# funcwj/setk

Measured on AMD Instinct MI355X. Metric: real-time-factor (audio-sec/wall-sec), 8-ch 16 kHz MVDR, higher is better.
Workload: dtype f32; 1 GPU; 8-ch 16 kHz oracle-mask MVDR, 30 s utterances, 125 per GPU (BASELINE configs[2] shard: 1000 at 8 GPUs), STFT 512/256/hann/center, inputs resident in HBM; utts_per_gpu=125, channels=8, frames=1876, beamformer=mvdr, parallelism=utterance-sharded x1

## Files before the change

setk_amd/csrc/fft512.h:

```cpp
#pragma once
#include <hip/hip_runtime.h>

namespace setk {

typedef float2 cf;

#define SETK_DEV __device__ __forceinline__

#define SETK_GLOBAL __attribute__((address_space(1)))
typedef const SETK_GLOBAL float* gcfloat_p;
typedef float v2f __attribute__((ext_vector_type(2)));
typedef const SETK_GLOBAL v2f* gcfloat2_p;
template <class T>
SETK_DEV const SETK_GLOBAL T* gptr(const T* p) {
    return (const SETK_GLOBAL T*)p;
}

SETK_DEV cf cadd(cf a, cf b) { return make_float2(a.x + b.x, a.y + b.y); }
SETK_DEV cf csub(cf a, cf b) { return make_float2(a.x - b.x, a.y - b.y); }
SETK_DEV cf cmul(cf a, cf b) {
    return make_float2(a.x * b.x - a.y * b.y, a.x * b.y + a.y * b.x);
}
SETK_DEV cf cmulc(cf a, cf b) {
    return make_float2(a.x * b.x + a.y * b.y, a.y * b.x - a.x * b.y);
}
SETK_DEV cf cconj(cf a) { return make_float2(a.x, -a.y); }
SETK_DEV cf cscale(cf a, float s) { return make_float2(a.x * s, a.y * s); }

__host__ __device__ constexpr int dft16_pos(int q) { return (q >> 2) + 4 * (q & 3); }

template <int DIR>
SETK_DEV void dft4(cf& a, cf& b, cf& c, cf& d) {
    cf s0 = cadd(a, c), s1 = csub(a, c), s2 = cadd(b, d), s3 = csub(b, d);
    cf r3 = DIR < 0 ? make_float2(s3.y, -s3.x) : make_float2(-s3.y, s3.x);
    a = cadd(s0, s2);
    c = csub(s0, s2);
    b = cadd(s1, r3);
    d = csub(s1, r3);
}

template <int DIR, int M>
SETK_DEV cf twid16(cf v) {
    constexpr float C1 = 0.92387953251128673848f;
    constexpr float S1 = 0.38268343236508978178f;
    constexpr float R2 = 0.70710678118654752440f;
    constexpr float D = (float)DIR;
    if constexpr (M == 1) return cmul(v, make_float2(C1, D * S1));
    if constexpr (M == 2) return make_float2(R2 * (v.x - D * v.y), R2 * (D * v.x + v.y));
    if constexpr (M == 3) return cmul(v, make_float2(S1, D * C1));
    if constexpr (M == 4) return make_float2(-D * v.y, D * v.x);
    if constexpr (M == 6) return make_float2(R2 * (-v.x - D * v.y), R2 * (D * v.x - v.y));
    if constexpr (M == 9) return cmul(v, make_float2(-C1, -D * S1));
    return v;
}

template <int DIR>
SETK_DEV void dft16(cf (&v)[16]) {
#pragma unroll
    for (int b = 0; b < 4; ++b) dft4<DIR>(v[b], v[4 + b], v[8 + b], v[12 + b]);
    v[4 * 1 + 1] = twid16<DIR, 1>(v[4 * 1 + 1]);
    v[4 * 2 + 1] = twid16<DIR, 2>(v[4 * 2 + 1]);
    v[4 * 3 + 1] = twid16<DIR, 3>(v[4 * 3 + 1]);
    v[4 * 1 + 2] = twid16<DIR, 2>(v[4 * 1 + 2]);
    v[4 * 2 + 2] = twid16<DIR, 4>(v[4 * 2 + 2]);
    v[4 * 3 + 2] = twid16<DIR, 6>(v[4 * 3 + 2]);
    v[4 * 1 + 3] = twid16<DIR, 3>(v[4 * 1 + 3]);
    v[4 * 2 + 3] = twid16<DIR, 6>(v[4 * 2 + 3]);
    v[4 * 3 + 3] = twid16<DIR, 9>(v[4 * 3 + 3]);
#pragma unroll
    for (int c = 0; c < 4; ++c)
        dft4<DIR>(v[4 * c], v[4 * c + 1], v[4 * c + 2], v[4 * c + 3]);
}

constexpr int kRow5 = 10;
__host__ __device__ constexpr int slot_entries(int row) { return 16 * row; }
__host__ __device__ constexpr int table_entries(int row) {
    return (row % 2 == 0) ? 2 * 16 * row + 16 * kRow5 : 640;
}
template <int ROW> struct LaneTab {
    static constexpr bool rows = (ROW % 2 == 0);
    static constexpr int estride = rows ? 1 : 16;
    static constexpr int lstride = rows ? ROW : 1;
    static constexpr int lstride5 = rows ? kRow5 : 1;
    static constexpr int size = rows ? 16 * ROW : 256;
};

template <int N, bool WIDE = true>
SETK_DEV void lds_row(const cf* row, cf (&out)[N]) {
    if (WIDE) {
        const float4* r4 = reinterpret_cast<const float4*>(__builtin_assume_aligned(row, 16));
#pragma unroll
        for (int n = 0; n < N / 2; ++n) {
            const float4 t = r4[n];
            out[2 * n] = make_float2(t.x, t.y);
            out[2 * n + 1] = make_float2(t.z, t.w);
        }
    } else {
#pragma unroll
        for (int n = 0; n < N; ++n) out[n] = row[n];
    }
}

template <int ROW>
SETK_DEV void fill_lane_tables(cf* win_l, cf* tw_l, cf* tw5_l, const float* window,
                               const float2* tw256, const float2* tw512, int tid, int nthreads) {
    for (int i = tid; i < 256; i += nthreads) {
        const int la = i & 15, j = i >> 4, n = la + 16 * j;
        typedef LaneTab<ROW> L;
        win_l[la * L::lstride + j * L::estride] = make_float2(window[2 * n], window[2 * n + 1]);
        tw_l[la * L::lstride + j * L::estride] = tw256[j * 16 + la];
    }
    for (int i = tid; i < 128; i += nthreads) {
        const int la = i & 15, m = i >> 4;
        tw5_l[la * LaneTab<ROW>::lstride5 + m * LaneTab<ROW>::estride] = tw512[la + 16 * m];
    }
}

template <int ROW>
SETK_DEV void apply_window(cf (&v)[16], const cf* win_row) {
    if (LaneTab<ROW>::rows) {
        const float4* w4 = reinterpret_cast<const float4*>(__builtin_assume_aligned(win_row, 16));
#pragma unroll
        for (int j = 0; j < 16; j += 2) {
            const float4 w = w4[j / 2];
            v[j] = make_float2(v[j].x * w.x, v[j].y * w.y);
            v[j + 1] = make_float2(v[j + 1].x * w.z, v[j + 1].y * w.w);
        }
    } else {
#pragma unroll
        for (int j = 0; j < 16; ++j) {
            const cf w = win_row[j * 16];
            v[j] = make_float2(v[j].x * w.x, v[j].y * w.y);
        }
    }
}

template <int DIR, int ROW, bool WIDE = (ROW % 2 == 0)>
SETK_DEV void fft256_stage_a_pad(cf (&v)[16], cf* slot, const cf* tw_row, int la) {
    dft16<DIR>(v);
    cf* dst = slot + la;
    if (WIDE) {
        const float4* w4 = reinterpret_cast<const float4*>(__builtin_assume_aligned(tw_row, 16));
#pragma unroll
        for (int q = 0; q < 16; q += 2) {
            const float4 w = w4[q / 2];
            cf t0 = v[dft16_pos(q)], t1 = v[dft16_pos(q + 1)];
            if (q) t0 = cmul(t0, make_float2(w.x, DIR > 0 ? -w.y : w.y));
            t1 = cmul(t1, make_float2(w.z, DIR > 0 ? -w.w : w.w));
            dst[q * ROW] = t0;
            dst[(q + 1) * ROW] = t1;
        }
    } else {
        cf wq[16];
        wq[1] = tw_row[16];
        wq[2] = tw_row[32];
#pragma unroll
        for (int q = 0; q < 16; ++q) {
            if (q + 3 < 16) wq[q + 3] = tw_row[(q + 3) * 16];
            cf t = v[dft16_pos(q)];
            if (q) {
                cf w = wq[q];
                if (DIR > 0) w.y = -w.y;
                t = cmul(t, w);
            }
            dst[q * ROW] = t;
        }
    }
}

template <int DIR, int ROW, bool WIDE = (ROW % 2 == 0)>
SETK_DEV void fft256_stage_b_pad(cf (&v)[16], const cf* slot, int la) {
    lds_row<16, WIDE>(slot + la * ROW, v);
    dft16<DIR>(v);
}

SETK_DEV void rfft_split(cf Zk, cf Zm, cf w, cf& Xk, cf& Xm) {
    cf A = make_float2(Zk.x + Zm.x, Zk.y - Zm.y);
    cf O = make_float2(Zk.y + Zm.y, Zm.x - Zk.x);
    cf B = cmul(w, O);
    Xk = cadd(A, B);
    Xm = make_float2(A.x - B.x, -(A.y - B.y));
}

SETK_DEV void irfft_merge(cf Yk, cf Ym, cf w, cf& Zk, cf& Zm) {
    cf E = make_float2(Yk.x + Ym.x, Yk.y - Ym.y);
    cf D = make_float2(Yk.x - Ym.x, Yk.y + Ym.y);
    cf O = cmulc(D, w);
    Zk = make_float2(E.x - O.y, E.y + O.x);
    Zm = make_float2(E.x + O.y, -E.y + O.x);
}

constexpr int kFrame = 512;

SETK_DEV int reflect_index(int i, int n) {
    if (i < 0) i = -i;
    if (i >= n) i = 2 * (n - 1) - i;
    return i;
}

template <class FloatPtr> struct RawPair;
template <> struct RawPair<gcfloat_p> {
    typedef gcfloat2_p ptr;
    static SETK_DEV cf get(ptr p, int i) {
        const v2f d = p[i];
        return make_float2(d.x, d.y);
    }
};
template <> struct RawPair<const float*> {
    typedef const float2* ptr;
    static SETK_DEV cf get(ptr p, int i) { return p[i]; }
};

template <class FloatPtr>
SETK_DEV void load_raw(cf (&v)[16], FloatPtr x, int n_samp, int s, int la, bool valid) {
    if (!valid) {
#pragma unroll
        for (int j = 0; j < 16; ++j) v[j] = make_float2(0.f, 0.f);
        return;
    }
    const bool interior = (s >= 0) && (s + kFrame <= n_samp) && ((((uintptr_t)(x + s)) & 7) == 0);
    if (interior) {
        typename RawPair<FloatPtr>::ptr p = (typename RawPair<FloatPtr>::ptr)(x + s);
#pragma unroll
        for (int j = 0; j < 16; ++j) v[j] = RawPair<FloatPtr>::get(p, la + 16 * j);
    } else {
#pragma unroll
        for (int j = 0; j < 16; ++j) {
            const int n = la + 16 * j;
            v[j] = make_float2(x[reflect_index(s + 2 * n, n_samp)],
                               x[reflect_index(s + 2 * n + 1, n_samp)]);
        }
    }
}

typedef const SETK_GLOBAL short* gcshort_p;
typedef const SETK_GLOBAL int* gcint_p;
SETK_DEV void load_raw_pcm(int (&v)[16], gcshort_p x, int n_samp, int s, int la, bool valid) {
    if (!valid) {
#pragma unroll
        for (int j = 0; j < 16; ++j) v[j] = 0;
        return;
    }
    const bool interior = (s >= 0) && (s + kFrame <= n_samp) && ((((uintptr_t)(x + s)) & 3) == 0);
    if (interior) {
        gcint_p p = (gcint_p)(x + s);
#pragma unroll
        for (int j = 0; j < 16; ++j) v[j] = p[la + 16 * j];
    } else {
#pragma unroll
        for (int j = 0; j < 16; ++j) {
            const int n = la + 16 * j;
            const int lo = x[reflect_index(s + 2 * n, n_samp)];
            const int hi = x[reflect_index(s + 2 * n + 1, n_samp)];
            v[j] = (lo & 0xffff) | (hi << 16);
        }
    }
}
SETK_DEV cf unpack_pcm(int v) { return make_float2((float)(short)(v & 0xffff), (float)(v >> 16)); }

SETK_DEV float qr_partner(float x) {
    int v = __builtin_bit_cast(int, x);
    v = __builtin_amdgcn_update_dpp(0, v, 0x140, 0xf, 0xf, true);
    v = __builtin_amdgcn_update_dpp(0, v, 0x121, 0xf, 0xf, true);
    return __builtin_bit_cast(float, v);
}

template <int ROW, bool WIDE = (ROW % 2 == 0)>
SETK_DEV void qr_stage23(cf* slot, float* nyq, const cf* tw5_row, int la) {
    cf v[16];
    fft256_stage_b_pad<-1, ROW, WIDE>(v, slot, la);
    const bool lane0 = (la == 0);
    cf* lo = slot + la;
    cf* mir = slot + (256 - 16 * 7) - la;
    cf t5[8];
    if (WIDE) {
        lds_row<8, true>(tw5_row, t5);
    } else {
        t5[0] = tw5_row[0];
        t5[1] = tw5_row[16];
    }
#pragma unroll
    for (int m = 0; m < 8; ++m) {
        if (!WIDE && m + 2 < 8) t5[m + 2] = tw5_row[16 * (m + 2)];
        const cf Zk = v[dft16_pos(m)];
        const cf src = v[dft16_pos(15 - m)];
        cf Zm = make_float2(qr_partner(src.x), qr_partner(src.y));
        const cf own = v[dft16_pos((16 - m) & 15)];
        Zm.x = lane0 ? own.x : Zm.x;
        Zm.y = lane0 ? own.y : Zm.y;
        cf Xk, Xm;
        rfft_split(Zk, Zm, t5[m], Xk, Xm);
        if (m == 0) {
            const cf Z128 = v[dft16_pos(8)];
            if (lane0) {
                slot[0] = make_float2(Xk.x, 0.f);
                *nyq = Xm.x;
                slot[128] = make_float2(2.f * Z128.x, -2.f * Z128.y);
            } else {
                lo[16 * m] = Xk;
                mir[16 * (7 - m)] = Xm;
            }
        } else {
            lo[16 * m] = Xk;
            mir[16 * (7 - m)] = Xm;
        }
    }
}

}
```

setk_amd/csrc/pass1.hip:

```cpp
#include "common.h"
#include "fft512.h"
#include "covar_fold.h"
#include <cstdio>
#include <type_traits>
#include <cstdlib>

namespace setk {

template <int C, bool DUMP, bool PCM = false>
__global__ __launch_bounds__(1024, 4) void stft_covar_kernel(Pass1Args a) {
    constexpr int NT = 1024;
    constexpr int TB = pass1_tile_frames(C);
    constexpr int NF = TB * C;
    constexpr int NP = npairs(C);
    constexpr int ND = PairSplit<C>::ND, NO = PairSplit<C>::NO;
    constexpr int NS = 32 / NF;
    constexpr int F = kBins, FP = kBinsPad;
    constexpr int ROW = 17;
    constexpr int SL = slot_entries(ROW);

    extern __shared__ __attribute__((aligned(16))) char smem[];
    cf* xt0 = reinterpret_cast<cf*>(smem);
    cf* win_l = xt0 + 2 * NF * SL;
    cf* tw_l = win_l + LaneTab<ROW>::size;
    cf* tw5_l = tw_l + LaneTab<ROW>::size;
    float* xn0 = reinterpret_cast<float*>(win_l + table_entries(ROW));
    float* nym = xn0 + 64;
    float* red = nym + 32;

    const int tid = threadIdx.x;
    const int wave = __builtin_amdgcn_readfirstlane(tid >> 6);
    const WorkItem wi = a.items[blockIdx.x];
    const UttDesc ud = a.utts[wi.utt];
    const int n_samp = ud.num_samples;
    const int T = ud.num_frames;
    const bool clamp = (a.flags & 0x2) != 0;
    const bool has_mn = ud.mask_n != nullptr;

    fill_lane_tables<ROW>(win_l, tw_l, tw5_l, a.window, a.tw256, a.tw512, tid, NT);

    float mx = 0.f;
    const int ct = tid - 512;
    const int f = ct & 255, q = (ct >> 8) & 1;
    float dg_s[ND], dg_n[ND];
    cf of_s[NO > 0 ? NO : 1], of_n[NO > 0 ? NO : 1];
    float aux0 = 0.f, aux1 = 0.f;
    const int ny_item = ct - 256;
    const bool ny_active = !DUMP && ny_item >= 0 && ny_item < 2 * NP + 2;

    if (wave < 8) {
        const int la = tid & 15, grp = tid >> 4;
        const int my_set = grp / NF;
        const int my_i = grp - my_set * NF;
        const int my_tt = my_i / C, my_c = my_i - my_tt * C;
        const bool producer = my_set < NS;
        gcfloat_p my_audio = gptr(ud.audio) + (size_t)my_c * n_samp;
        gcshort_p my_pcm = (gcshort_p)gptr(ud.audio) + (size_t)my_c * ud.ch_stride;
        const cf* win_row = win_l + la * LaneTab<ROW>::lstride;
        const cf* tw_row = tw_l + la * LaneTab<ROW>::lstride;
        const cf* tw5_row = tw5_l + la * LaneTab<ROW>::lstride5;
        const bool ny_lane = !DUMP && producer && my_c == 0 && la == 0;

        typename std::conditional<PCM, int, cf>::type raw[16];
        float raw_ms = 0.f, raw_mn = 0.f;
        bool raw_ok = false, raw_last = false;
        auto fetch = [&](int tb_tile) {
            const int t = tb_tile + my_tt;
            raw_ok = t < wi.t1;
            raw_last = t == T - 1;
            if constexpr (PCM) load_raw_pcm(raw, my_pcm, n_samp, t * a.g.hop - a.g.pad, la, raw_ok);
            else load_raw(raw, my_audio, n_samp, t * a.g.hop - a.g.pad, la, raw_ok);
            if (ny_lane) {
                raw_ms = 0.f;
                raw_mn = 0.f;
                if (raw_ok) {
                    raw_ms = gptr(ud.mask_s)[(size_t)t * F + 256];
                    if (has_mn) raw_mn = gptr(ud.mask_n)[(size_t)t * F + 256];
                }
            }
        };
        const bool half_max = a.g.hop <= kNfft / 2;
        auto produce = [&](int b, int tb_next_own) {
            cf* slot = xt0 + (b * NF + my_i) * SL;
            cf v[16];
#pragma unroll
            for (int j = 0; j < 16; ++j) {
                if constexpr (PCM) v[j] = unpack_pcm(raw[j]);
                else v[j] = raw[j];
            }
#pragma unroll
            for (int j = 0; j < 8; ++j) mx = max3_abs(mx, v[j].x, v[j].y);
            if (!half_max || raw_last) {
#pragma unroll
                for (int j = 8; j < 16; ++j) mx = max3_abs(mx, v[j].x, v[j].y);
            }
            apply_window<ROW>(v, win_row);
            if (ny_lane) {
                const float s = clamp ? fminf(raw_ms, 1.f) : raw_ms;
                nym[(b * 2 + 0) * 8 + my_tt] = s;
                nym[(b * 2 + 1) * 8 + my_tt] = raw_ok ? (has_mn ? raw_mn : 1.f - s) : 0.f;
            }
            fft256_stage_a_pad<-1, ROW>(v, slot, tw_row, la);
            __builtin_amdgcn_wave_barrier();
            if (tb_next_own < wi.t1) fetch(tb_next_own);
            qr_stage23<ROW>(slot, xn0 + b * 32 + my_i, tw5_row, la);
        };

        wg_barrier();
        if (producer) fetch(wi.t0 + my_set * TB);
        if (producer && my_set == 0) produce(0, wi.t0 + NS * TB);
        wg_barrier();
        int buf = 0, next_set = 1 % NS;
#pragma unroll 1
        for (int tb = wi.t0; tb < wi.t1; tb += TB, buf ^= 1) {
            const bool prod = producer && (my_set == next_set) && (tb + TB < wi.t1);
            next_set = (next_set + 1 == NS) ? 0 : next_set + 1;
            if (prod) produce(buf ^ 1, tb + TB + NS * TB);
            wg_barrier();
        }
    } else {
#pragma unroll
        for (int e = 0; e < ND; ++e) dg_s[e] = dg_n[e] = 0.f;
#pragma unroll
        for (int e = 0; e < NO; ++e) {
            of_s[e] = make_float2(0.f, 0.f);
            of_n[e] = make_float2(0.f, 0.f);
        }
        int ny_i = 0, ny_j = 0;
        {
            const int e = (ny_item < NP) ? ny_item : ny_item - NP;
            int cnt = 0;
#pragma unroll
            for (int i = 0; i < C; ++i)
#pragma unroll
                for (int j = i; j < C; ++j) {
                    if (cnt == e) { ny_i = i; ny_j = j; }
                    ++cnt;
                }
        }
        float cur_s[TB], cur_n[TB], nxt_s[TB], nxt_n[TB];
        auto fetch_masks = [&](int tb_tile, float (&ms)[TB], float (&mn)[TB]) {
#pragma unroll
            for (int tt = 0; tt < TB; ++tt) {
                const int t = tb_tile + tt;
                float vs = 0.f, vn = 0.f;
                if (t < wi.t1) {
                    vs = gptr(ud.mask_s)[(size_t)t * F + f];
                    if (has_mn) vn = gptr(ud.mask_n)[(size_t)t * F + f];
                }
                ms[tt] = vs;
                mn[tt] = vn;
            }
        };
        if (!DUMP) fetch_masks(wi.t0, cur_s, cur_n);
        wg_barrier();
        wg_barrier();
        int buf = 0;
#pragma unroll 1
        for (int tb = wi.t0; tb < wi.t1; tb += TB, buf ^= 1) {
            const cf* xt = xt0 + buf * NF * SL;
            const float* xn = xn0 + buf * 32;
            if (DUMP) {
                for (int i = q; i < NF; i += 2) {
                    const int tt = i / C, c = i - tt * C;
                    const int t = tb + tt;
                    if (t < wi.t1) {
                        float2* base = a.spec_dump ? reinterpret_cast<float2*>(a.spec_dump)
                                                   : reinterpret_cast<float2*>(ud.wave_out);
                        float2* dst = base + ((size_t)c * T + t) * (a.dump_pitch ? a.dump_pitch : F);
                        dst[f] = xt[i * SL + f];
                        if (f == 0) dst[256] = make_float2(xn[i], 0.f);
                    }
                }
            } else {
                if (tb + TB < wi.t1) fetch_masks(tb + TB, nxt_s, nxt_n);
#pragma unroll
                for (int tt = 0; tt < TB; ++tt) {
                    cf x[C];
#pragma unroll
                    for (int c = 0; c < C; ++c) x[c] = xt[(tt * C + c) * SL + f];
                    const bool fvalid = tb + tt < wi.t1;
                    const float ws = clamp ? fminf(cur_s[tt], 1.f) : cur_s[tt];
                    const float wn = fvalid ? (has_mn ? cur_n[tt] : 1.f - ws) : 0.f;
                    if (q == 0) {
                        aux0 += ws;
                        aux1 += wn;
                        accumulate_half<C, 0>(x, ws, wn, dg_s, dg_n, of_s, of_n);
                    } else {
                        accumulate_half<C, 1>(x, ws, wn, dg_s, dg_n, of_s, of_n);
                    }
                    if (ny_active) {
                        const float prod_ny =
                            (ny_item < 2 * NP) ? xn[tt * C + ny_i] * xn[tt * C + ny_j] : 1.f;
                        const bool speech = (ny_item < NP) || (ny_item == 2 * NP);
                        const float w256 = nym[(buf * 2 + (speech ? 0 : 1)) * 8 + tt];
                        aux0 = fmaf(w256, prod_ny, aux0);
                    }
                }
#pragma unroll
                for (int tt = 0; tt < TB; ++tt) {
                    cur_s[tt] = nxt_s[tt];
                    cur_n[tt] = nxt_n[tt];
                }
            }
            wg_barrier();
        }
    }

    if (!DUMP) {
        if (wi.last) {
            const int covered = (T - 1) * a.g.hop - a.g.pad + kNfft;
            for (int c = 0; c < C; ++c)
                for (int i = covered + tid; i < n_samp; i += NT) {
                    if constexpr (PCM)
                        mx = fmaxf(mx, fabsf((float)((gcshort_p)gptr(ud.audio))[(size_t)c * ud.ch_stride + i]));
                    else
                        mx = fmaxf(mx, fabsf(gptr(ud.audio)[(size_t)c * n_samp + i]));
                }
        }
        if constexpr (PCM) mx *= 3.0517578125e-05f;
#pragma unroll
        for (int o = 32; o > 0; o >>= 1) mx = fmaxf(mx, __shfl_xor(mx, o));
        if ((tid & 63) == 0) red[tid >> 6] = mx;
        __syncthreads();
        if (tid == 0) {
            float bm = red[0];
#pragma unroll
            for (int w = 1; w < NT / 64; ++w) bm = fmaxf(bm, red[w]);
            atomicMax(a.norm_bits + wi.utt, __float_as_uint(bm));
        }
        if (wave >= 8) {
            float* P = a.partials + (size_t)wi.part * nplanes_partial(C) * FP;
            if (q == 0) {
                store_half<C, 0>(P, f, dg_s, dg_n, of_s, of_n);
                P[(4 * NP + 0) * FP + f] = aux0;
                P[(4 * NP + 1) * FP + f] = aux1;
            } else {
                store_half<C, 1>(P, f, dg_s, dg_n, of_s, of_n);
            }
            if (ny_active) {
                if (ny_item < NP) {
                    P[(0 * NP + ny_item) * FP + 256] = aux0;
                    P[(1 * NP + ny_item) * FP + 256] = 0.f;
                } else if (ny_item < 2 * NP) {
                    P[(2 * NP + ny_item - NP) * FP + 256] = aux0;
                    P[(3 * NP + ny_item - NP) * FP + 256] = 0.f;
                } else {
                    P[(4 * NP + ny_item - 2 * NP) * FP + 256] = aux0;
                }
            }
        }
    }
}

constexpr int kBmFrames = 64;
constexpr int kBmSlot = slot_entries(17) + 1;

__global__ __launch_bounds__(1024, 4) void stft_binmajor_kernel(Pass1Args a, int C) {
    constexpr int ROW = 17;
    constexpr int NT = 1024;
    extern __shared__ __attribute__((aligned(16))) char smem[];
    cf* xt = reinterpret_cast<cf*>(smem);
    cf* win_l = xt + kBmFrames * kBmSlot;
    cf* tw_l = win_l + LaneTab<ROW>::size;
    cf* tw5_l = tw_l + LaneTab<ROW>::size;
    float* xn = reinterpret_cast<float*>(win_l + table_entries(ROW));

    const int tid = threadIdx.x;
    const int wave = tid >> 6, lane = tid & 63;
    const int la = tid & 15, grp = tid >> 4;
    const WorkItem wi = a.items[blockIdx.x];
    const UttDesc ud = a.utts[wi.utt];
    const int n_samp = ud.num_samples, T = ud.num_frames;
    const int Tp = (T + 3) & ~3;
    cf* out = reinterpret_cast<cf*>(ud.wave_out);
    fill_lane_tables<ROW>(win_l, tw_l, tw5_l, a.window, a.tw256, a.tw512, tid, NT);
    const cf* win_row = win_l + la * LaneTab<ROW>::lstride;
    const cf* tw_row = tw_l + la * LaneTab<ROW>::lstride;
    const cf* tw5_row = tw5_l + la * LaneTab<ROW>::lstride5;
    cf* slot = xt + grp * kBmSlot;
    const int t = wi.t0 + grp;
    const bool valid = t < wi.t1;

    const int s0 = t * a.g.hop - a.g.pad;
    __syncthreads();
    for (int c = 0; c < C; ++c) {
        cf v[16];
        load_raw(v, gptr(ud.audio) + (size_t)c * n_samp, n_samp, s0, la, valid);
        apply_window<ROW>(v, win_row);
        fft256_stage_a_pad<-1, ROW>(v, slot, tw_row, la);
        __builtin_amdgcn_wave_barrier();
        qr_stage23<ROW>(slot, xn + grp, tw5_row, la);
        __syncthreads();
        {
            const int fr = 2 * (lane & 31), half = lane >> 5;
            const int t2 = wi.t0 + fr;
            for (int f = 2 * wave + half; f < kBins; f += 2 * (NT / 64)) {
                cf v0, v1;
                if (f < 256) {
                    v0 = xt[fr * kBmSlot + f];
                    v1 = xt[(fr + 1) * kBmSlot + f];
                } else {
                    v0 = make_float2(xn[fr], 0.f);
                    v1 = make_float2(xn[fr + 1], 0.f);
                }
                cf* dst = out + ((size_t)f * C + c) * Tp + t2;
                if (t2 + 1 < wi.t1)
                    *reinterpret_cast<float4*>(dst) = make_float4(v0.x, v0.y, v1.x, v1.y);
                else if (t2 < wi.t1)
                    *dst = v0;
            }
        }
        __syncthreads();
    }
}

hipError_t launch_stft_binmajor(int C, const Pass1Args& a, int n_items, hipStream_t s) {
    const size_t lds = (size_t)kBmFrames * kBmSlot * sizeof(cf) + table_entries(17) * sizeof(cf) +
                       kBmFrames * sizeof(float);
    hipError_t e = hipFuncSetAttribute(reinterpret_cast<const void*>(stft_binmajor_kernel),
                                       hipFuncAttributeMaxDynamicSharedMemorySize, (int)lds);
    if (e != hipSuccess) return e;
    hipLaunchKernelGGL(stft_binmajor_kernel, dim3(n_items), dim3(1024), lds, s, a, C);
    return hipGetLastError();
}

template <int C, bool DUMP, bool PCM = false>
static hipError_t launch_pass1_t(const Pass1Args& a, int n_items, hipStream_t s) {
    constexpr int NF = pass1_tile_frames(C) * C;
    const size_t lds = (size_t)2 * NF * slot_entries(17) * sizeof(cf) + table_entries(17) * sizeof(cf) +
                       (64 + 32 + 16) * sizeof(float);
    auto k = stft_covar_kernel<C, DUMP, PCM>;
    hipError_t e = hipFuncSetAttribute(reinterpret_cast<const void*>(k),
                                       hipFuncAttributeMaxDynamicSharedMemorySize, (int)lds);
    if (e != hipSuccess) return e;
    hipLaunchKernelGGL(k, dim3(n_items), dim3(1024), lds, s, a);
    return hipGetLastError();
}

hipError_t launch_pass1(int C, bool dump, const Pass1Args& a, int n_items, hipStream_t s, bool pcm16) {
    if (pcm16 && dump) return hipErrorInvalidValue;
#define SETK_CASE(c)                                                \
    case c:                                                         \
        if (dump) return launch_pass1_t<c, true>(a, n_items, s);     \
        if (pcm16) return launch_pass1_t<c, false, true>(a, n_items, s); \
        return launch_pass1_t<c, false>(a, n_items, s);
    switch (C) {
        SETK_CASE(1)
        SETK_CASE(2)
        SETK_CASE(3)
        SETK_CASE(4)
        SETK_CASE(5)
        SETK_CASE(6)
        SETK_CASE(7)
        SETK_CASE(8)
    }
#undef SETK_CASE
    return hipErrorInvalidValue;
}

__global__ __launch_bounds__(320) void covar_finalize_kernel(FinalizeArgs a) {
    const int f = threadIdx.x;
    const int u = blockIdx.z;
    const int C = a.num_channels;
    const int NP = npairs(C);
    const int planes_in = 4 * NP + 2;
    const int planes_out = a.with_ry ? 6 * NP : 4 * NP;
    const int e = blockIdx.y;
    if (f >= kBinsPad) return;
    const UttDesc ud = a.utts[u];
    float* out = a.covar + ((size_t)u * planes_out + e) * kBinsPad;
    if (f >= kBins) {
        out[f] = 0.f;
        return;
    }
    const float* P = a.partials + (size_t)ud.part0 * planes_in * kBinsPad;
    const size_t slab = (size_t)planes_in * kBinsPad;
    if (e < 4 * NP) {
        const int sel = e / (2 * NP);
        float acc = 0.f, den = 0.f;
        for (int p = 0; p < ud.nparts; ++p) {
            acc += P[p * slab + (size_t)e * kBinsPad + f];
            den += P[p * slab + (size_t)(4 * NP + sel) * kBinsPad + f];
        }
        const float sc = a.num_scale / fmaxf(den, 1e-6f);
        out[f] = acc * sc;
    } else {
        const int r = e - 4 * NP;
        float acc = 0.f;
        for (int p = 0; p < ud.nparts; ++p)
            acc += P[p * slab + (size_t)r * kBinsPad + f] +
                   P[p * slab + (size_t)(2 * NP + r) * kBinsPad + f];
        const float sc = a.num_scale / fmaxf((float)ud.num_frames, 1e-6f);
        out[f] = acc * sc;
    }
}

hipError_t launch_finalize(const FinalizeArgs& a, int n_utts, hipStream_t s) {
    const int NP = npairs(a.num_channels);
    const int planes_out = a.with_ry ? 6 * NP : 4 * NP;
    dim3 grid(1, planes_out, n_utts);
    hipLaunchKernelGGL(covar_finalize_kernel, grid, dim3(320), 0, s, a);
    return hipGetLastError();
}

}
```

Baseline: 2.109 million x real time (audio seconds per wall second, all GPUs).

## Stream contiguous frame ranges per producer group to reuse overlapping STFT halves

When there is one producer set and hop is half the FFT size, each producer group now walks its own contiguous run of frames. Each frame reuses the previous frame's second half from registers and loads only a new half-frame, which halves audio loads and per-frame max work. The mask fetch stride and the frame-valid checks are changed to match the new frame-to-slot mapping. Covariance-thread state and the partial-result stores move into the consumer branch, which should lower register pressure for the producer waves. The cost is more branching, plus a frame ordering that depends on hop and tile count.

```diff
diff --git a/setk_amd/csrc/fft512.h b/setk_amd/csrc/fft512.h
--- a/setk_amd/csrc/fft512.h
+++ b/setk_amd/csrc/fft512.h
@@ -253,6 +253,48 @@
             const int lo = x[reflect_index(s + 2 * n, n_samp)];
             const int hi = x[reflect_index(s + 2 * n + 1, n_samp)];
             v[j] = (lo & 0xffff) | (hi << 16);
+        }
+    }
+}
+template <class FloatPtr>
+SETK_DEV void load_half(cf (&h)[8], FloatPtr x, int n_samp, int s, int la, bool valid) {
+    if (!valid) {
+#pragma unroll
+        for (int j = 0; j < 8; ++j) h[j] = make_float2(0.f, 0.f);
+        return;
+    }
+    const bool interior = (s >= 0) && (s + kFrame / 2 <= n_samp) && ((((uintptr_t)(x + s)) & 7) == 0);
+    if (interior) {
+        typename RawPair<FloatPtr>::ptr p = (typename RawPair<FloatPtr>::ptr)(x + s);
+#pragma unroll
+        for (int j = 0; j < 8; ++j) h[j] = RawPair<FloatPtr>::get(p, la + 16 * j);
+    } else {
+#pragma unroll
+        for (int j = 0; j < 8; ++j) {
+            const int n = la + 16 * j;
+            h[j] = make_float2(x[reflect_index(s + 2 * n, n_samp)],
+                               x[reflect_index(s + 2 * n + 1, n_samp)]);
+        }
+    }
+}
+SETK_DEV void load_half_pcm(int (&h)[8], gcshort_p x, int n_samp, int s, int la, bool valid) {
+    if (!valid) {
+#pragma unroll
+        for (int j = 0; j < 8; ++j) h[j] = 0;
+        return;
+    }
+    const bool interior = (s >= 0) && (s + kFrame / 2 <= n_samp) && ((((uintptr_t)(x + s)) & 3) == 0);
+    if (interior) {
+        gcint_p p = (gcint_p)(x + s);
+#pragma unroll
+        for (int j = 0; j < 8; ++j) h[j] = p[la + 16 * j];
+    } else {
+#pragma unroll
+        for (int j = 0; j < 8; ++j) {
+            const int n = la + 16 * j;
+            const int lo = x[reflect_index(s + 2 * n, n_samp)];
+            const int hi = x[reflect_index(s + 2 * n + 1, n_samp)];
+            h[j] = (lo & 0xffff) | (hi << 16);
         }
     }
 }
diff --git a/setk_amd/csrc/pass1.hip b/setk_amd/csrc/pass1.hip
--- a/setk_amd/csrc/pass1.hip
+++ b/setk_amd/csrc/pass1.hip
@@ -6,6 +6,8 @@
 #include <cstdlib>
 
 namespace setk {
+
+constexpr bool kRequestAtTop = true;
 
 template <int C, bool DUMP, bool PCM = false>
 __global__ __launch_bounds__(1024, 4) void stft_covar_kernel(Pass1Args a) {
@@ -36,18 +38,13 @@
     const int T = ud.num_frames;
     const bool clamp = (a.flags & 0x2) != 0;
     const bool has_mn = ud.mask_n != nullptr;
+    constexpr bool kStreams = !DUMP && NS == 1;
+    const bool streams = kStreams && a.g.hop == kNfft / 2;
+    const int n_tiles = (wi.t1 - wi.t0 + TB - 1) / TB;
 
     fill_lane_tables<ROW>(win_l, tw_l, tw5_l, a.window, a.tw256, a.tw512, tid, NT);
 
     float mx = 0.f;
-    const int ct = tid - 512;
-    const int f = ct & 255, q = (ct >> 8) & 1;
-    float dg_s[ND], dg_n[ND];
-    cf of_s[NO > 0 ? NO : 1], of_n[NO > 0 ? NO : 1];
-    float aux0 = 0.f, aux1 = 0.f;
-    const int ny_item = ct - 256;
-    const bool ny_active = !DUMP && ny_item >= 0 && ny_item < 2 * NP + 2;
-
     if (wave < 8) {
         const int la = tid & 15, grp = tid >> 4;
         const int my_set = grp / NF;
@@ -107,6 +104,87 @@
         };
 
         wg_barrier();
+        if (streams) {
+            const int my_t0 = wi.t0 + my_tt * n_tiles;
+            const int my_end = min(wi.t1, my_t0 + n_tiles);
+            typedef typename std::conditional<PCM, int, cf>::type raw_t;
+            raw_t hx[8], hy[8];
+            float ny_s = 0.f, ny_n = 0.f;
+            auto fetch_half = [&](raw_t (&h)[8], int t, bool ok) {
+                const int s = t * (kNfft / 2) - a.g.pad + kNfft / 2;
+                if constexpr (PCM) load_half_pcm(h, my_pcm, n_samp, s, la, ok);
+                else load_half(h, my_audio, n_samp, s, la, ok);
+            };
+            auto fetch_ny = [&](int t, bool ok) {
+                if (ny_lane) {
+                    ny_s = 0.f;
+                    ny_n = 0.f;
+                    if (ok) {
+                        ny_s = gptr(ud.mask_s)[(size_t)t * F + 256];
+                        if (has_mn) ny_n = gptr(ud.mask_n)[(size_t)t * F + 256];
+                    }
+                }
+            };
+            auto unpack = [&](raw_t r) {
+                if constexpr (PCM) return unpack_pcm(r);
+                else return r;
+            };
+            auto produce_s = [&](int b, int t, raw_t (&h0)[8], raw_t (&h1)[8]) {
+                cf* slot = xt0 + (b * NF + my_i) * SL;
+                const bool ok = t < my_end;
+                const float ms = ny_s, mn = ny_n;
+                cf v[16];
+#pragma unroll
+                for (int j = 0; j < 8; ++j) {
+                    v[j] = unpack(h0[j]);
+                    v[j + 8] = unpack(h1[j]);
+                }
+                auto request = [&]() {
+                    fetch_half(h0, t + 1, t + 1 < my_end);
+                    fetch_ny(t + 1, t + 1 < my_end);
+                };
+                if (kRequestAtTop) request();
+                if (!ok) {
+#pragma unroll
+                    for (int j = 0; j < 8; ++j) v[j] = make_float2(0.f, 0.f);
+                }
+#pragma unroll
+                for (int j = 8; j < 16; ++j) mx = max3_abs(mx, v[j].x, v[j].y);
+                apply_window<ROW>(v, win_row);
+                if (ny_lane) {
+                    const float s = clamp ? fminf(ms, 1.f) : ms;
+                    nym[(b * 2 + 0) * 8 + my_tt] = s;
+                    nym[(b * 2 + 1) * 8 + my_tt] = ok ? (has_mn ? mn : 1.f - s) : 0.f;
+                }
+                fft256_stage_a_pad<-1, ROW>(v, slot, tw_row, la);
+                __builtin_amdgcn_wave_barrier();
+                if (!kRequestAtTop) request();
+                qr_stage23<ROW>(slot, xn0 + b * 32 + my_i, tw5_row, la);
+            };
+            if (producer) {
+                const bool ok = my_t0 < my_end;
+                fetch_half(hx, my_t0 - 1, ok);
+                fetch_half(hy, my_t0, ok);
+                fetch_ny(my_t0, ok);
+#pragma unroll
+                for (int j = 0; j < 8; ++j) {
+                    const cf u = unpack(hx[j]);
+                    mx = max3_abs(mx, u.x, u.y);
+                }
+            }
+            int b0 = 0;
+#pragma unroll 1
+            for (int k = 0; k < n_tiles; k += 2) {
+                asm volatile("" : "+s"(b0));
+                if (producer) produce_s(b0, my_t0 + k, hx, hy);
+                wg_barrier();
+                if (k + 1 < n_tiles) {
+                    if (producer) produce_s(b0 ^ 1, my_t0 + k + 1, hy, hx);
+                    wg_barrier();
+                }
+            }
+            wg_barrier();
+        } else {
         if (producer) fetch(wi.t0 + my_set * TB);
         if (producer && my_set == 0) produce(0, wi.t0 + NS * TB);
         wg_barrier();
@@ -118,7 +196,15 @@
             if (prod) produce(buf ^ 1, tb + TB + NS * TB);
             wg_barrier();
         }
+        }
     } else {
+        const int ct = tid - 512;
+        const int f = ct & 255, q = (ct >> 8) & 1;
+        float dg_s[ND], dg_n[ND];
+        cf of_s[NO > 0 ? NO : 1], of_n[NO > 0 ? NO : 1];
+        float aux0 = 0.f, aux1 = 0.f;
+        const int ny_item = ct - 256;
+        const bool ny_active = !DUMP && ny_item >= 0 && ny_item < 2 * NP + 2;
 #pragma unroll
         for (int e = 0; e < ND; ++e) dg_s[e] = dg_n[e] = 0.f;
 #pragma unroll
@@ -139,10 +225,12 @@
                 }
         }
         float cur_s[TB], cur_n[TB], nxt_s[TB], nxt_n[TB];
-        auto fetch_masks = [&](int tb_tile, float (&ms)[TB], float (&mn)[TB]) {
+        const int fstep = streams ? n_tiles : 1;
+        const int bstep = streams ? 1 : TB;
+        auto fetch_masks = [&](int base, float (&ms)[TB], float (&mn)[TB]) {
 #pragma unroll
             for (int tt = 0; tt < TB; ++tt) {
-                const int t = tb_tile + tt;
+                const int t = base + tt * fstep;
                 float vs = 0.f, vn = 0.f;
                 if (t < wi.t1) {
                     vs = gptr(ud.mask_s)[(size_t)t * F + f];
@@ -157,7 +245,7 @@
         wg_barrier();
         int buf = 0;
 #pragma unroll 1
-        for (int tb = wi.t0; tb < wi.t1; tb += TB, buf ^= 1) {
+        for (int tb = wi.t0, tile = 0; tile < n_tiles; tb += bstep, ++tile, buf ^= 1) {
             const cf* xt = xt0 + buf * NF * SL;
             const float* xn = xn0 + buf * 32;
             if (DUMP) {
@@ -173,13 +261,13 @@
                     }
                 }
             } else {
-                if (tb + TB < wi.t1) fetch_masks(tb + TB, nxt_s, nxt_n);
+                if (tile + 1 < n_tiles) fetch_masks(tb + bstep, nxt_s, nxt_n);
 #pragma unroll
                 for (int tt = 0; tt < TB; ++tt) {
                     cf x[C];
 #pragma unroll
                     for (int c = 0; c < C; ++c) x[c] = xt[(tt * C + c) * SL + f];
-                    const bool fvalid = tb + tt < wi.t1;
+                    const bool fvalid = tb + tt * fstep < wi.t1;
                     const float ws = clamp ? fminf(cur_s[tt], 1.f) : cur_s[tt];
                     const float wn = fvalid ? (has_mn ? cur_n[tt] : 1.f - ws) : 0.f;
                     if (q == 0) {
@@ -205,6 +293,27 @@
             }
             wg_barrier();
         }
+        if (!DUMP) {
+            float* P = a.partials + (size_t)wi.part * nplanes_partial(C) * FP;
+            if (q == 0) {
+                store_half<C, 0>(P, f, dg_s, dg_n, of_s, of_n);
+                P[(4 * NP + 0) * FP + f] = aux0;
+                P[(4 * NP + 1) * FP + f] = aux1;
+            } else {
+                store_half<C, 1>(P, f, dg_s, dg_n, of_s, of_n);
+            }
+            if (ny_active) {
+                if (ny_item < NP) {
+                    P[(0 * NP + ny_item) * FP + 256] = aux0;
+                    P[(1 * NP + ny_item) * FP + 256] = 0.f;
+                } else if (ny_item < 2 * NP) {
+                    P[(2 * NP + ny_item - NP) * FP + 256] = aux0;
+                    P[(3 * NP + ny_item - NP) * FP + 256] = 0.f;
+                } else {
+                    P[(4 * NP + ny_item - 2 * NP) * FP + 256] = aux0;
+                }
+            }
+        }
     }
 
     if (!DUMP) {
@@ -228,27 +337,6 @@
 #pragma unroll
             for (int w = 1; w < NT / 64; ++w) bm = fmaxf(bm, red[w]);
             atomicMax(a.norm_bits + wi.utt, __float_as_uint(bm));
-        }
-        if (wave >= 8) {
-            float* P = a.partials + (size_t)wi.part * nplanes_partial(C) * FP;
-            if (q == 0) {
-                store_half<C, 0>(P, f, dg_s, dg_n, of_s, of_n);
-                P[(4 * NP + 0) * FP + f] = aux0;
-                P[(4 * NP + 1) * FP + f] = aux1;
-            } else {
-                store_half<C, 1>(P, f, dg_s, dg_n, of_s, of_n);
-            }
-            if (ny_active) {
-                if (ny_item < NP) {
-                    P[(0 * NP + ny_item) * FP + 256] = aux0;
-                    P[(1 * NP + ny_item) * FP + 256] = 0.f;
-                } else if (ny_item < 2 * NP) {
-                    P[(2 * NP + ny_item - NP) * FP + 256] = aux0;
-                    P[(3 * NP + ny_item - NP) * FP + 256] = 0.f;
-                } else {
-                    P[(4 * NP + ny_item - 2 * NP) * FP + 256] = aux0;
-                }
-            }
         }
     }
 }
```

After: 2.022 million x real time (audio seconds per wall second, all GPUs). -4.1%, worse.
